# emanuele-artioli/elvis

Hardware: AMD Instinct MI355X
Metric: restored 1080p frames/sec, SinSR 4x path (ELVIS v2 Downsample) (higher is better)
Workload: dtype f16; 1 GPU; 30-frame 1920x1080 synthetic clip per GPU, ELVIS v2 Downsample (SinSR 4x), block 8, levels 0-3, weights seed 0 (random init), quantize=True; frames_per_gpu=30, parallelism=single GPU, gn_fused_into_conv=True, frames_per_invocation=15

## Files before the change

elvis_amd/_lib.py:

```python
from __future__ import annotations

import ctypes as C
import os
import threading
from typing import Optional

HERE = os.path.dirname(os.path.abspath(__file__))
LIBPATH = os.environ.get("ELVIS_AMD_LIB") or os.path.join(HERE, "lib", "libelvis_amd.so")

F32, F16 = 0, 1
ROUND_CV2, ROUND_HALF_UP = 0, 1

_lock = threading.Lock()
_lib: Optional[C.CDLL] = None

vp, i32, f32, i64, f64 = C.c_void_p, C.c_int, C.c_float, C.c_longlong, C.c_double


class ConvDesc(C.Structure):
    _fields_ = [(n, C.c_int) for n in (
        "dtype", "n", "h", "w", "cin", "cin_pitch", "cin2", "cin2_pitch", "cout", "cout_pitch",
        "ksize", "stride", "pad_before", "upsample", "ho", "wo", "act", "prologue", "subpixel")]


SIGNATURES = {
    "elvis_abi_version": [],
    "elvis_last_error": [],
    "elvis_last_launch": [],
    "elvis_recompose_u8": [vp, vp, vp, vp, vp, i32, i32, i32, i32, i32, i32, i32, i32, i32, vp],
    "elvis_area_downscale_u8": [vp, vp, i32, i32, i32, i32, i32, i32, vp],
    "elvis_blend_u8": [vp, vp, vp, vp, i32, i32, i32, i32, i32, i32, i32, f32, vp],
    "elvis_select_levels_u8": [vp, vp, i32, vp, vp, i32, i32, i32, i32, i32, i32, i32, vp],
    "elvis_tile_accumulate_f32": [vp, vp, vp, vp, vp, vp, i32, i32, i32, i32, i32, i32, i32, f32, vp],
    "elvis_tile_normalize_u8": [vp, vp, vp, i32, i32, i32, vp],
    "elvis_sse_u8": [vp, vp, vp, vp, vp, i32, i32, i32, i32, vp],
    "elvis_block_ssim_u8": [vp, vp, vp, vp, i32, i32, i32, i32, i32, vp],
    "elvis_u8_to_float": [vp, vp, i32, i32, i32, i32, i32, f32, f32, i32, i32, vp],
    "elvis_float_to_u8": [vp, i32, vp, vp, i32, i32, i32, i32, f32, f32, i32, i32, vp],
    "elvis_conv_packed_weight_bytes": [C.POINTER(ConvDesc)],
    "elvis_conv_pack_weights": [C.POINTER(ConvDesc), vp, vp, vp],
    "elvis_conv2d": [C.POINTER(ConvDesc), vp, vp, vp, vp, vp, i32, vp, vp, vp, vp, vp],
    "elvis_conv_stats_tiles": [C.POINTER(ConvDesc)],
    "elvis_conv_kernel_name": [C.POINTER(ConvDesc), C.c_char_p, C.c_size_t],
    "elvis_conv_kernel_name_for_call": [C.POINTER(ConvDesc), i32, i32, C.c_char_p, C.c_size_t],
    "elvis_conv_x3_eligible": [C.POINTER(ConvDesc)],
    "elvis_conv_debug_set": [C.c_char_p, i32],
    "elvis_gn_partials_to_sums": [vp, i32, i32, i32, vp, i32, i32, vp],
    "elvis_groupnorm_workspace_floats": [i32, i32, i32, i32],
    "elvis_groupnorm_sums": [vp, i32, i32, i32, i32, i32, vp, i32, i32, vp, vp],
    "elvis_groupnorm_affine": [vp, vp, vp, vp, vp, vp, vp, i32, i32, i32, i32, f32, vp],
    "elvis_affine_act": [vp, vp, i32, i32, i32, i32, i32, i32, vp, vp, i32, vp],
    "elvis_layernorm": [vp, vp, i32, i64, i32, i32, i32, vp, vp, f32, vp],
    "elvis_swin_packed_bytes": [i32, i32, i32],
    "elvis_swin_pack_weights": [vp, vp, vp, i32, i32, i32, vp],
    "elvis_swin_mlp": [vp, vp, vp, vp, vp, vp, vp, i64, i32, i32, i32, i32, f32, vp],
    "elvis_swin_ln_linear": [vp, vp, vp, vp, vp, vp, i64, i32, i32, i32, i32, f32, vp],
    "elvis_swin_pack_proj_mlp": [vp, vp, vp, vp, i32, i32, vp],
    "elvis_swin_proj_mlp": [vp, vp, vp, vp, vp, vp, vp, vp, vp, i64, i32, i32, i32, i32, i32, f32, vp],
    "elvis_window_attention": [vp, vp, i32, i32, i32, i32, i32, i32, i32, i32, i32, i32, vp, f32, vp],
    "elvis_bicubic_upsample": [vp, vp, i32, i32, i32, i32, i32, i32, i32, i32, vp],
    "elvis_vq_nearest": [vp, vp, vp, i32, i64, i32, i32, i32, vp, i32, vp],
    "elvis_pad_reflect_axpy": [vp, vp, i32, i32, i32, i32, i32, i32, i32, i32, i32, i32, f32, vp, f32, vp],
    "elvis_crop_copy": [vp, vp, i32, i32, i32, i32, i32, i32, i32, i32, i32, vp],
    "elvis_convert_act": [vp, i32, vp, i32, i64, i32, vp],
    "elvis_degrade_downsample_u8": [vp, vp, vp, i32, i32, i32, i32, i32, i32, i32, vp],
    "elvis_degrade_gaussian_u8": [vp, vp, vp, i32, i32, i32, i32, i32, i32, i32, f32, f32, f32, vp],
    "elvis_degrade_dct_u8": [vp, vp, vp, vp, vp, i32, i32, i32, i32, i32, i32, i32, vp],
    "elvis_degrade_scale_u8": [vp, vp, vp, i32, i32, i32, i32, i32, i32, i32, vp, vp, vp, i32, vp],
    "elvis_degrade_gaussian_fx_u8": [vp, vp, vp, i32, i32, i32, i32, i32, i32, i32, i32, i32, i32, vp],
    "elvis_classical_lanczos_u8": [vp, vp, vp, i32, i32, i32, i32, i32, i32, i32, vp, vp],
    "elvis_classical_unsharp_u8": [vp, vp, vp, i32, i32, i32, i32, i32, i32, i32, i32, vp, vp, i32, vp],
    "elvis_temporal_blend_u8": [vp, vp, i32, i64, f64, f64, vp],
    "elvis_block_gather_u8": [vp, vp, vp, vp, i32, i32, i32, i32, i32, i32, i32, i32, i32, vp],
    "elvis_shrink_select_topk": [vp, vp, vp, i32, i32, i32, i32, vp],
    "elvis_shrink_passes_plan": [i32, i32, i32, i32, vp, vp, vp, i32],
    "elvis_shrink_select_passes": [vp, vp, vp, vp, vp, vp, i32, i32, i32, i32, i32, i32, i32, vp],
    "elvis_stretch_index": [vp, vp, i32, i32, i32, i32, i32, i32, vp],
    "elvis_dcnv2": [vp, vp, vp, vp, vp, i32, i32, i32, i32, i32, i32, i32, i32, i32, i32, i32, i32, vp],
    "elvis_temporal_stack": [vp, vp, i32, i32, i32, i32, i32, i32, i32, i32, vp],
    "elvis_plane_merge": [vp, vp, vp, i32, i32, i32, i32, i32, i32, vp],
}


def lib() -> C.CDLL:
    global _lib
    if _lib is not None:
        return _lib
    with _lock:
        if _lib is not None:
            return _lib
        if not os.path.exists(LIBPATH):
            raise RuntimeError(
                f"libelvis_amd.so not found at {LIBPATH}. Build it with `python -m elvis_amd._build` "
                "(needs hipcc). There is no CPU fallback for the restoration path.")
        import torch
        try:
            handle = C.CDLL(LIBPATH)
        except OSError as exc:
            raise RuntimeError(f"failed to load {LIBPATH}: {exc}") from exc
        for name, argtypes in SIGNATURES.items():
            fn = getattr(handle, name)
            fn.argtypes = argtypes
            fn.restype = C.c_int
        handle.elvis_last_error.restype = C.c_char_p
        handle.elvis_last_launch.restype = C.c_char_p
        handle.elvis_conv_packed_weight_bytes.restype = C.c_size_t
        handle.elvis_groupnorm_workspace_floats.restype = C.c_size_t
        handle.elvis_swin_packed_bytes.restype = C.c_size_t
        if handle.elvis_abi_version() != 1:
            raise RuntimeError("libelvis_amd.so ABI version mismatch")
        _lib = handle
    return _lib


def check(rc: int, device=None) -> None:
    if rc == 0:
        return
    msg = lib().elvis_last_error().decode("utf-8", "replace")
    if rc == -1:
        raise ValueError(msg)
    label = str(device) if device is not None else "unknown device"
    raise RuntimeError(f"elvis_amd kernel failed on {label}: {msg}")


def ptr(t) -> int:
    return 0 if t is None else t.data_ptr()


def stream_handle(device=None) -> int:
    import torch
    return torch.cuda.current_stream(device).cuda_stream


def require_gpu(device) -> None:
    import torch
    dev = torch.device(device)
    if dev.type != "cuda":
        raise RuntimeError(
            f"elvis_amd runs on MI355X only (got device '{dev}'); there is no CPU path in the product. "
# ... 13 lines not shown
```

elvis_amd/csrc/conv.hip:

```cpp
#include "conv_kernels.inc"
#include "conv_ws.inc"
#include <string.h>

__attribute__((visibility("hidden"))) int elvis_conv_launch_f32_(const void* conv_args, int halo, int tco, int id, hipStream_t stream, void* query);
__attribute__((visibility("hidden"))) int elvis_conv_pack_x3p_(const float* w_oihw, void* packed, int cout, int ctot, int nkc, int n_co_tiles,
                                                              int tco, int taps, hipStream_t stream);

#include <atomic>
static std::atomic<int> g_no_halo{0};
static bool no_halo() { return g_no_halo.load(std::memory_order_relaxed) > 0; }
extern "C" int elvis_conv_debug_set(const char* key, int value) {
    ELVIS_REQUIRE(key, "elvis_conv_debug_set: null key");
    if (!strcmp(key, "no_halo")) { g_no_halo.store(value, std::memory_order_relaxed); return ELVIS_OK; }
    ELVIS_REQUIRE(false, "elvis_conv_debug_set: unknown key '%s'", key);
}

static void conv_geom(const elvis_conv_desc* d, int* nkc1, int* nkc, int* co_pad) {
    int kc = kc_of(d);
    *nkc1 = (d->cin + kc - 1) / kc;
    *nkc = *nkc1 + (d->cin2 > 0 ? (d->cin2 + kc - 1) / kc : 0);
    TileCfg t = choose_tile(d->cout);
    *co_pad = ((d->cout + t.tco - 1) / t.tco) * t.tco;
}

extern "C" size_t elvis_conv_packed_weight_bytes(const elvis_conv_desc* d) {
    if (!d || d->cin <= 0 || d->cout <= 0) return 0;
    int nkc1, nkc, co_pad;
    conv_geom(d, &nkc1, &nkc, &co_pad);
    return (size_t)d->ksize * d->ksize * nkc * co_pad * (x3_planar_fmt(d) ? 128 : 64);
}

extern "C" int elvis_conv_pack_weights(const elvis_conv_desc* d, const float* w_oihw, void* packed,
                                       elvis_stream_t stream) {
    int rc = validate(d);
    if (rc) return rc;
    ELVIS_REQUIRE(w_oihw && packed, "elvis_conv_pack_weights: null pointer");
    int nkc1, nkc, co_pad;
    conv_geom(d, &nkc1, &nkc, &co_pad);
    if (x3_planar_fmt(d)) {
        const int tco = choose_tile(d->cout).tco;
        return elvis_conv_pack_x3p_(w_oihw, packed, d->cout, d->cin + d->cin2, nkc, co_pad / tco, tco, d->ksize * d->ksize, (hipStream_t)stream);
    }
    int KC = kc_elems(d->dtype);
    long long total = (long long)d->ksize * d->ksize * nkc * co_pad * KC;
    int grid = (int)((total + 255) / 256);
    int ctot = d->cin + d->cin2;
// ... 18 lines not shown
}

enum class ConvPath { WS, HALO, IGEMM };
static ConvPath conv_path(const elvis_conv_desc* d, bool has_residual, bool has_stats) {
    if (no_halo()) return ConvPath::IGEMM;
    if (ws_shape_ok(d) && !has_residual && !has_stats) return ConvPath::WS;
    return halo_eligible(d) ? ConvPath::HALO : ConvPath::IGEMM;
}

static int conv_walk(const elvis_conv_desc* d, ConvPath path, const ConvArgs& a, hipStream_t stream, ConvPick* query) {
    const TileCfg t = choose_tile(d->cout);
    const bool f16 = d->dtype == ELVIS_F16;
    if (path == ConvPath::WS) return dispatch_ws(a, t.tco, stream, query);
    if (path == ConvPath::IGEMM) return f16 ? dispatch<half_t>(a, t.id, stream, query) : elvis_conv_launch_f32_(&a, 0, t.tco, t.id, stream, query);
    if (!f16) return elvis_conv_launch_f32_(&a, 1, t.tco, t.id, stream, query);
    switch (t.tco) {
        case 128: return launch_halo<half_t, 128>(a, stream, query);
        case 64: return launch_halo<half_t, 64>(a, stream, query);
        case 32: return launch_halo<half_t, 32>(a, stream, query);
        default: return launch_halo<half_t, 16>(a, stream, query);
    }
}

static int conv_plan(const elvis_conv_desc* d, ConvPath path, ConvArgs& a, ConvPick& pick) {
    a.n = d->n; a.h = d->h; a.w_in = d->w;
    a.cin = d->cin; a.cin_pitch = d->cin_pitch; a.cin2 = d->cin2; a.cin2_pitch = d->cin2_pitch;
    a.cout = d->cout; a.cout_pitch = d->cout_pitch;
    a.ksize = d->ksize; a.stride = d->stride; a.pad = d->pad_before; a.upsample = d->upsample;
    a.ho = d->ho; a.wo = d->wo; a.act = d->act; a.prologue = d->prologue;
    conv_geom(d, &a.nkc1, &a.nkc, &a.co_pad);
    TileCfg t = choose_tile(d->cout);
    a.M = (long long)d->n * d->ho * d->wo;
    a.n_co_tiles = a.co_pad / t.tco;
    a.n_px_tiles = (a.M + t.tpx - 1) / t.tpx;
    const bool s2d = d->ksize == 2 && d->subpixel == ELVIS_CONV_S2D;
    const bool subpix = d->ksize == 2 && !s2d;
    a.sub = d->ksize == 2;
    a.par_a = subpix ? (d->subpixel - 1) >> 1 : 0;
    a.par_b = subpix ? (d->subpixel - 1) & 1 : 0;
    a.ostr = subpix ? 2 : 1;
    a.pad2y = subpix ? 1 - a.par_a : (s2d ? d->pad_before : 0);
    a.pad2x = subpix ? 1 - a.par_b : (s2d ? d->pad_before : 0);
    a.s2d = s2d ? 1 : 0;
    a.istr = s2d ? 2 : 1;
    a.nkc_c = s2d ? d->cin / 4 / kc_of(d) : 0x3fffffff;
    a.wfull = d->w;
    if (s2d) {
        a.h = d->ho;
        a.w_in = d->wo;
    }
    a.x3 = d->dtype == ELVIS_F32X3 ? (x3_planar_run(d) ? 2 : 1) : 0;
    a.two = (halo_two(d) || halo_g1(d)) ? 1 : 0;
    a.tall = (halo_two(d) && halo_tall(d)) ? 1 : 0;
    int rc = conv_walk(d, path, a, nullptr, &pick);
    if (rc) return rc;
    a.tiles_x = ((subpix ? d->w : d->wo) + HALO_TX - 1) / HALO_TX;
    a.tiles_y = pick.ty > 0 ? ((subpix ? d->h : d->ho) + pick.ty - 1) / pick.ty : 0;
    a.strip = HALO_STRIP < a.tiles_x ? HALO_STRIP : 0;
    a.strip_full = a.strip > 0 ? a.tiles_x / a.strip : 0;
    return ELVIS_OK;
}

extern "C" int elvis_conv_stats_tiles(const elvis_conv_desc* d) {
    if (!d || !halo_eligible(d)) return 0;
    ConvArgs a{};
    ConvPick pick{};
    if (conv_plan(d, ConvPath::HALO, a, pick)) return 0;
    return d->n * a.tiles_y * a.tiles_x;
}

extern "C" int elvis_conv_kernel_name_for_call(const elvis_conv_desc* d, int has_residual, int has_stats, char* buf, size_t n) {
    int rc = validate(d);
    if (rc) return rc;
    ELVIS_REQUIRE(buf && n > 0, "elvis_conv_kernel_name: null buffer");
    ConvArgs a{};
    ConvPick pick{};
    rc = conv_plan(d, conv_path(d, has_residual != 0, has_stats != 0), a, pick);
    if (rc) return rc;
    snprintf(buf, n, "%s", pick.name);
    return ELVIS_OK;
}

extern "C" int elvis_conv_kernel_name(const elvis_conv_desc* d, char* buf, size_t n) {
    return elvis_conv_kernel_name_for_call(d, 0, 0, buf, n);
}

extern "C" int elvis_conv2d(const elvis_conv_desc* d, const void* x, const void* x2, const void* w_packed,
                            const float* bias, const void* residual, int residual_pitch, const float* pa,
                            const float* pb, void* out, float* stats, elvis_stream_t stream) {
    int rc = validate(d);
    if (rc) return rc;
    ELVIS_REQUIRE(x && w_packed && out, "elvis_conv2d: null pointer");
    ELVIS_REQUIRE(d->cin2 == 0 || x2, "elvis_conv2d: cin2 > 0 but x2 is null");
    ELVIS_REQUIRE(!d->prologue || (pa && pb), "elvis_conv2d: prologue requested without pa/pb");
    ELVIS_REQUIRE(d->dtype != ELVIS_F32X3 || x3_eligible(d),
                  "elvis_conv2d: this shape has no compensated-f16 kernel (elvis_conv_x3_eligible): run it as ELVIS_F32");
    ELVIS_REQUIRE(!residual || residual_pitch >= d->cout, "elvis_conv2d: bad residual pitch");
    ELVIS_REQUIRE(((uintptr_t)x | (uintptr_t)(x2 ? x2 : x) | (uintptr_t)w_packed | (uintptr_t)out) % 16 == 0,
                  "elvis_conv2d: pointers must be 16-byte aligned");
    const ConvPath path = conv_path(d, residual != nullptr, stats != nullptr);
    ELVIS_REQUIRE(path != ConvPath::IGEMM || !stats, "elvis_conv2d: fused statistics need a 3x3/stride-1 conv with cout >= 64 (query elvis_conv_stats_tiles)");
    ELVIS_REQUIRE(path == ConvPath::IGEMM || (long long)d->n * d->h * d->w < 0x7fffffffLL, "conv: input too large for 32-bit pixel indices");
    ConvArgs a{};
    ConvPick pick{};
    rc = conv_plan(d, path, a, pick);
    if (rc) return rc;
    a.x = x; a.x2 = x2; a.w = w_packed; a.bias = bias; a.res = residual; a.pa = pa; a.pb = pb; a.out = out;
    a.res_pitch = residual_pitch; a.stats = stats;
    return conv_walk(d, path, a, (hipStream_t)stream, nullptr);
}
```

elvis_amd/csrc/conv_kernels.inc:

```
#pragma once
#include "common.h"

#ifndef ELVIS_CONV_HOOKS
#define ELVIS_STAGE(x) x
#define ELVIS_STAGE_W(x) x
#define ELVIS_STAGE_H(x) x
#define ELVIS_SETPRIO(x)
#define ELVIS_BARRIER() __syncthreads()
#define ELVIS_HOOK_SKIP_STORE(tv)
#define ELVIS_HOOK_STAMP_BEGIN
#define ELVIS_HOOK_STAMP_LOOP
#define ELVIS_HOOK_STAMP_EPILOGUE
#define ELVIS_HOOK_STAMP_END
#endif

namespace {

struct ConvArgs {
    const void* x;
    const void* x2;
    const void* w;
    const float* bias;
    const void* res;
    const float* pa;
    const float* pb;
    void* out;
    int n, h, w_in;
    int cin, cin_pitch, cin2, cin2_pitch;
    int cout, cout_pitch, res_pitch;
    int ksize, stride, pad, upsample;
    int ho, wo;
    int act, prologue;
    int nkc;
    int nkc1;
    int co_pad;
    long long M;
    int n_co_tiles;
    long long n_px_tiles;
    int two, tall;
    float* stats;
    int tiles_x, tiles_y;
    int sub, par_a, par_b;
    int ostr, pad2y, pad2x;
    int s2d, istr, nkc_c, wfull;
    int strip;
    int strip_full;
    int x3;
};

struct ConvPick {
    const char* name;
    int ty;
    int set(const char* name_, int ty_) { name = name_; ty = ty_; return ELVIS_OK; }
};
constexpr const char* tf(bool b) { return b ? "true" : "false"; }

template <typename T> struct Frag;
template <> struct Frag<half_t> { typedef half8 type; };
template <> struct Frag<float> { typedef float4v type; };

__device__ __forceinline__ void mma_tile(float4v& acc, const half8& a, const half8& b) {
    acc = __builtin_amdgcn_mfma_f32_16x16x32_f16(a, b, acc, 0, 0, 0);
}
__device__ __forceinline__ void mma_tile(float4v& acc, const float4v& a, const float4v& b) {
    acc = __builtin_amdgcn_mfma_f32_16x16x4f32(a[0], b[0], acc, 0, 0, 0);
    acc = __builtin_amdgcn_mfma_f32_16x16x4f32(a[1], b[1], acc, 0, 0, 0);
    acc = __builtin_amdgcn_mfma_f32_16x16x4f32(a[2], b[2], acc, 0, 0, 0);
    acc = __builtin_amdgcn_mfma_f32_16x16x4f32(a[3], b[3], acc, 0, 0, 0);
}

__device__ __forceinline__ unsigned x3_pair(float v) {
    const half_t h = (half_t)v;
    const half_t l = (half_t)(v - (float)h);
    return (unsigned)__builtin_bit_cast(unsigned short, h) | ((unsigned)__builtin_bit_cast(unsigned short, l) << 16);
}
__device__ __forceinline__ uint4 x3_pair4(uint4 v) {
    return make_uint4(x3_pair(__builtin_bit_cast(float, v.x)), x3_pair(__builtin_bit_cast(float, v.y)),
                      x3_pair(__builtin_bit_cast(float, v.z)), x3_pair(__builtin_bit_cast(float, v.w)));
}
template <bool X3> __device__ __forceinline__ void mma_tile_x(float4v& acc, const half8& a, const half8& b) { mma_tile(acc, a, b); }
template <bool X3> __device__ __forceinline__ void mma_tile_x(float4v& acc, const float4v& a, const float4v& b) {
    if constexpr (X3) {
        const uint4 ap = __builtin_bit_cast(uint4, a);
        const uint4 a1 = make_uint4(__builtin_amdgcn_perm(ap.x, ap.x, 0x01000100u), __builtin_amdgcn_perm(ap.y, ap.y, 0x01000100u),
                                    __builtin_amdgcn_perm(ap.z, ap.z, 0x01000100u), __builtin_amdgcn_perm(ap.w, ap.w, 0x01000100u));
        const uint4 a2 = make_uint4(ap.x >> 16, ap.y >> 16, ap.z >> 16, ap.w >> 16);
        const half8 B = __builtin_bit_cast(half8, b);
        acc = __builtin_amdgcn_mfma_f32_16x16x32_f16(__builtin_bit_cast(half8, a1), B, acc, 0, 0, 0);
        acc = __builtin_amdgcn_mfma_f32_16x16x32_f16(__builtin_bit_cast(half8, a2), B, acc, 0, 0, 0);
    } else {
        mma_tile(acc, a, b);
    }
}

template <typename F> __device__ __forceinline__ F lds_frag(const char* p) {
    return *reinterpret_cast<const F*>(__builtin_assume_aligned(p, 16));
}

__device__ __forceinline__ int lds_row_off(int row, int q) {
    return row * 64 + ((q ^ (((row >> 2) & 1) << 1)) << 4);
}

constexpr int G1_NST128 = 3, G1_NST64 = 2;
typedef __attribute__((address_space(3))) void* lds_ptr_t;
typedef const __attribute__((address_space(1))) void* glb_ptr_t;

template <typename T> struct PrologueVec { float a[DT<T>::VEC], b[DT<T>::VEC]; };
template <typename T> __device__ __forceinline__ uint4 prologue_apply(uint4 v, const float (&pa)[DT<T>::VEC], const float (&pb)[DT<T>::VEC]);
template <> __device__ __forceinline__ uint4 prologue_apply<float>(uint4 v, const float (&pa)[4], const float (&pb)[4]) {
    float* f = reinterpret_cast<float*>(&v);
#pragma unroll
    for (int i = 0; i < 4; ++i) {
        float t = fmaf(f[i], pa[i], pb[i]);
        f[i] = t / (1.0f + expf(-t));
    }
    return v;
}
template <> __device__ __forceinline__ uint4 prologue_apply<half_t>(uint4 v, const float (&pa)[8], const float (&pb)[8]) {
    half_t* hv = reinterpret_cast<half_t*>(&v);
#pragma unroll
    for (int i = 0; i < 8; ++i) {
        float t = fmaf((float)hv[i], pa[i], pb[i]);
        hv[i] = (half_t)(t * __builtin_amdgcn_rcpf(1.0f + __expf(-t)));
    }
    return v;
}

__device__ __forceinline__ unsigned prologue_dword_f16(unsigned w, float a0, float a1, float b0, float b1, float K) {
    float u0, u1, e1;
    asm volatile(
        "v_fma_mix_f32 %1, %0, %4, %6 op_sel:[0,0,0] op_sel_hi:[1,0,0]\n\t"
        "v_fma_mix_f32 %2, %0, %5, %7 op_sel:[1,0,0] op_sel_hi:[1,0,0]\n\t"
        "v_exp_f32 %0, %1\n\t"
        "v_exp_f32 %3, %2\n\t"
        "v_fma_f32 %0, %0, %8, %8\n\t"
// ... 300 lines not shown
        }
    }
}

template <typename T, int TCO, int NT, int TY, bool PRO, int KS, bool ACT, bool X3>
__device__ __forceinline__ void conv3x3_halo_body(const ConvArgs& p) {
    constexpr int TX = 32, HX = TX + KS - 1, HY = TY + KS - 1, HP = HX * HY;
    constexpr bool TWO = NT == 256;
    constexpr int NSLOT = (TWO || KS == 2) ? 2 : 3;
    constexpr int NHB = TWO ? 1 : 2;
    constexpr bool WDMA = TWO;
    constexpr bool G1 = TWO && KS == 1;
    constexpr bool PSC = TWO && PRO && sizeof(T) == 2;
    constexpr int G1_NST = TCO == 64 ? G1_NST64 : G1_NST128;
    constexpr int HCH = HP * 4;
    constexpr int H_PER = (HCH + NT - 1) / NT;
    constexpr int HALO_BYTES = HP * 64;
    constexpr int W_TAP_BYTES = TCO * 64;
    constexpr int W_BYTES = KS * W_TAP_BYTES;
    constexpr int W_CHUNKS = W_TAP_BYTES / 16;
    constexpr int W_PER = (W_CHUNKS + NT - 1) / NT;
    constexpr int NW_CO = TCO >= 64 ? TCO / 64 : 1, NW_PX = (NT / 64) / NW_CO;
    constexpr int ROWS = TY / NW_PX;
    constexpr int WPX = ROWS * 2, WCO = TCO >= 64 ? 4 : TCO / 16;
    constexpr int VEC = DT<T>::VEC, KC = 4 * VEC;
    typedef typename Frag<T>::type frag_t;
    static_assert(ROWS * NW_PX == TY && ROWS >= 1, "tile rows must split evenly over the pixel waves");

    extern __shared__ __attribute__((aligned(16))) char smem[];
    char* const halo = smem;
    char* const wring = smem + NHB * HALO_BYTES;
    float* const ptab = reinterpret_cast<float*>(smem + NHB * HALO_BYTES + NSLOT * W_BYTES);

    const unsigned nblk = (unsigned)p.n_co_tiles * (unsigned)p.tiles_x * (unsigned)p.tiles_y * (unsigned)p.n;
    unsigned bid = blockIdx.x;
    {
        const unsigned q = nblk >> 3, r = nblk & 7u;
        const unsigned xcd = bid & 7u, idx = bid >> 3;
        bid = (xcd < r ? xcd * (q + 1) : r * (q + 1) + (xcd - r) * q) + idx;
    }
    int co_tile = 0;
    unsigned t = bid;
    if (p.n_co_tiles > 1) {
        t = bid / (unsigned)p.n_co_tiles;
        co_tile = (int)(bid - t * (unsigned)p.n_co_tiles);
    }
    int tx, ty, nimg;
    if (p.strip > 0) {
        const unsigned per_img = (unsigned)p.tiles_x * (unsigned)p.tiles_y;
        const unsigned ni = t / per_img;
        unsigned r = t - ni * per_img;
        const unsigned full = (unsigned)p.strip_full, strip_tiles = (unsigned)p.strip * (unsigned)p.tiles_y;
        unsigned s = r / strip_tiles;
        unsigned sw = (unsigned)p.strip;
        if (s >= full) { s = full; sw = (unsigned)p.tiles_x - full * (unsigned)p.strip; }
        r -= s * strip_tiles;
        const unsigned y = r / sw;
        nimg = (int)ni;
        ty = (int)y;
        tx = (int)(s * (unsigned)p.strip + (r - y * sw));
    } else {
        const unsigned row = t / (unsigned)p.tiles_x;
        tx = (int)(t - row * (unsigned)p.tiles_x);
        const unsigned ni = row / (unsigned)p.tiles_y;
        ty = (int)(row - ni * (unsigned)p.tiles_y);
        nimg = (int)ni;
    }
    const int oy0 = ty * TY, ox0 = tx * TX, co0 = co_tile * TCO;

    const int tid = threadIdx.x, lane = tid & 63, wave = tid >> 6;
    ELVIS_HOOK_STAMP_BEGIN
    const int w_co = wave / NW_PX, w_px = wave % NW_PX;
    const int lh = p.upsample ? p.h * 2 : p.h, lw = p.upsample ? p.w_in * 2 : p.w_in;

    const int pad_y = KS == 2 ? p.pad2y : KS / 2, pad_x = KS == 2 ? p.pad2x : KS / 2;
    int h_src[H_PER];
    unsigned h_ok = 0;
#pragma unroll
    for (int i = 0; i < H_PER; ++i) {
        int chunk = tid + i * NT;
        int pix = chunk >> 2;
        int hy = pix / HX, hx = pix - hy * HX;
        int gy = oy0 + hy - pad_y, gx = ox0 + hx - pad_x;
        bool ok = chunk < HCH && gy >= 0 && gy < lh && gx >= 0 && gx < lw;
        int sy = p.upsample ? (gy >> 1) : gy, sx = p.upsample ? (gx >> 1) : gx;
        h_src[i] = ok ? ((nimg * p.h + sy) * p.istr * p.w_in + sx) * p.istr : 0;
        h_ok |= (ok ? 1u : 0u) << i;
    }
    const bool halo_inside = oy0 - pad_y >= 0 && oy0 - pad_y + HY <= lh && ox0 - pad_x >= 0 && ox0 - pad_x + HX <= lw &&
                             (p.cin % KC) == 0 && (p.cin2 % KC) == 0 && p.cin_pitch >= p.nkc1 * KC && !(KS == 2 && p.s2d);
    const int q4 = tid & 3;
    const int nkc = p.nkc;
    const int nrows = nkc * KS;

    constexpr int HA = (H_PER + 1) / 2;
    uint4 hreg[H_PER];

    int wl_off[W_PER];
#pragma unroll
    for (int i = 0; i < W_PER; ++i) {
        int chunk = tid + i * NT;
        wl_off[i] = lds_row_off(chunk >> 2, chunk & 3);
    }

    auto chunk_c0 = [&](int kc, int& pixoff) -> int {
        pixoff = 0;
        if (KS == 2 && p.s2d) {
            const int ph = kc / p.nkc_c;
            pixoff = (ph >> 1) * p.wfull + (ph & 1);
            return (kc - ph * p.nkc_c) * KC + q4 * VEC;
        }
        return (kc >= p.nkc1 ? kc - p.nkc1 : kc) * KC + q4 * VEC;
    };
    auto halo_load = [&](int kc, int i0, int i1, bool live = true) {
        const bool second = kc >= p.nkc1;
        const char* xsrc = (const char*)(second ? p.x2 : p.x);
        const int pitch = second ? p.cin2_pitch : p.cin_pitch;
        int pixoff;
        const int c0 = chunk_c0(kc, pixoff);
        const int c0c = c0 < pitch ? c0 : 0;
// ... 10 lines not shown
        const bool ch_ok = c0 < pitch;
        char* dst = halo + buf * HALO_BYTES;
        float la[VEC], lb[VEC];
        if (PRO) {
            const float* tp = ptab + (kc * 4 + q4) * 2 * VEC;
#pragma unroll
            for (int e = 0; e < VEC; e += 4) {
                float4v a4 = *reinterpret_cast<const float4v*>(tp + e);
                float4v b4 = *reinterpret_cast<const float4v*>(tp + VEC + e);
#pragma unroll
                for (int k = 0; k < 4; ++k) { la[e + k] = a4[k]; lb[e + k] = b4[k]; }
            }
        }
#pragma unroll
        for (int i = i0; i < i1; ++i) {
            uint4 v = hreg[i];
            if constexpr (PSC) {
                const float K = -1.4426950408889634f;
                v.x = prologue_dword_f16(v.x, la[0], la[1], lb[0], lb[1], K);
                v.y = prologue_dword_f16(v.y, la[2], la[3], lb[2], lb[3], K);
                v.z = prologue_dword_f16(v.z, la[4], la[5], lb[4], lb[5], K);
                v.w = prologue_dword_f16(v.w, la[6], la[7], lb[6], lb[7], K);
            } else if (PRO) {
                v = prologue_apply<T>(v, la, lb);
            }
            if constexpr (X3) v = x3_pair4(v);
            if (!halo_inside) {
                const bool keep = ch_ok && ((h_ok >> i) & 1u);
                v.x = keep ? v.x : 0u; v.y = keep ? v.y : 0u; v.z = keep ? v.z : 0u; v.w = keep ? v.w : 0u;
            }
            int chunk = tid + i * NT;
            if ((i + 1) * NT <= HCH || chunk < HCH)
                *reinterpret_cast<uint4*>(dst + lds_row_off(chunk >> 2, chunk & 3)) = v;
        }
    };
    auto halo_act = [&](int kc, int slot, int half) {
        constexpr int HV = VEC / 2;
        const float* tp = ptab + (kc * 4 + q4) * 2 * VEC + half * HV;
        float a[HV], b[HV];
#pragma unroll
        for (int e = 0; e < HV; e += 2) {
            float2 a2 = *reinterpret_cast<const float2*>(tp + e);
            float2 b2 = *reinterpret_cast<const float2*>(tp + VEC + e);
            a[e] = a2.x; a[e + 1] = a2.y; b[e] = b2.x; b[e + 1] = b2.y;
        }
        uint2 v = half ? make_uint2(hreg[slot].z, hreg[slot].w) : make_uint2(hreg[slot].x, hreg[slot].y);
        v = prologue_apply_half(v, a, b, T());
        if (half) { hreg[slot].z = v.x; hreg[slot].w = v.y; } else { hreg[slot].x = v.x; hreg[slot].y = v.y; }
    };
    auto halo_write = [&](int kc, int buf, int slot) {
        const bool second = kc >= p.nkc1;
        const int pitch = second ? p.cin2_pitch : p.cin_pitch;
        int pixoff_;
        const int c0 = chunk_c0(kc, pixoff_);
        const bool keep = c0 < pitch && ((h_ok >> slot) & 1u);
        uint4 v = hreg[slot];
        if constexpr (X3) v = x3_pair4(v);
        v.x = keep ? v.x : 0u; v.y = keep ? v.y : 0u; v.z = keep ? v.z : 0u; v.w = keep ? v.w : 0u;
        int chunk = tid + slot * NT;
        if ((slot + 1) * NT <= HCH || chunk < HCH)
            *reinterpret_cast<uint4*>(halo + buf * HALO_BYTES + lds_row_off(chunk >> 2, chunk & 3)) = v;
    };
    static_assert(W_PER <= 2, "weight staging holds at most two 16-byte chunks per thread per tap");
    constexpr bool W_FULL0 = W_CHUNKS >= NT, W_FULL1 = W_PER == 2 && W_CHUNKS >= 2 * NT;
    const bool w_ok0 = W_FULL0 || tid < W_CHUNKS, w_ok1 = W_PER == 2 && (W_FULL1 || tid + NT < W_CHUNKS);
    uint4 wr00 = {}, wr01 = {}, wr10 = {}, wr11 = {}, wr20 = {}, wr21 = {};
// ... 648 lines not shown
        }
    } else
    if (p.stats) {
        float* red = reinterpret_cast<float*>(smem);
#pragma unroll
        for (int i = 0; i < WCO; ++i)
#pragma unroll
            for (int r = 0; r < 4; ++r) {
                const float a = row16_sum(st[i][r]), b = row16_sum(sq[i][r]);
                if (lr == 0) {
                    int cl = w_co * (16 * WCO) + cgrp * WCO + i * 4 + r;
                    red[(w_px * TCO + cl) * 2 + 0] = a;
                    red[(w_px * TCO + cl) * 2 + 1] = b;
                }
            }
        __syncthreads();
        if (tid < TCO && co0 + tid < p.cout) {
            float a = 0.f, b = 0.f;
#pragma unroll
            for (int w = 0; w < NW_PX; ++w) {
                a += red[(w * TCO + tid) * 2 + 0];
                b += red[(w * TCO + tid) * 2 + 1];
            }
            long long tile = ((long long)nimg * p.tiles_y + ty) * p.tiles_x + tx;
            float* dst = p.stats + (tile * p.cout + co0 + tid) * 2;
            dst[0] = a;
            dst[1] = b;
        }
    }
    ELVIS_HOOK_STAMP_END
}

template <typename T, int TCO, int NT, int TY, bool PRO, int KS = 3, bool ACT = false>
__global__ __launch_bounds__(NT, 2) void conv3x3_halo_kernel(ConvArgs p) {
    conv3x3_halo_body<T, TCO, NT, TY, PRO, KS, ACT, false>(p);
}
template <int TCO, int TY, bool PRO, int KS = 3, bool ACT = false>
__global__ __launch_bounds__(512, 2) void conv3x3_halo_x3_kernel(ConvArgs p) {
    conv3x3_halo_body<float, TCO, 512, TY, PRO, KS, ACT, true>(p);
}

struct TileCfg {
    int tco, tpx, id;
};
inline TileCfg choose_tile(int cout) {
    if (cout % 128 == 0) return {128, 128, 0};
    if (cout >= 64) return {64, 128, 1};
    if (cout <= 16) return {16, 256, 3};
    return {32, 256, 2};
}
inline bool halo_eligible(const elvis_conv_desc* d) {
    if (d->ksize == 2) return true;
    bool same = d->ho == (d->upsample ? 2 * d->h : d->h) && d->wo == (d->upsample ? 2 * d->w : d->w);
    if (d->ksize == 3) return d->stride == 1 && d->pad_before == 1 && same;
    return d->ksize == 1 && d->stride == 1 && d->pad_before == 0 && same && !d->prologue &&
           (long long)d->ho * d->wo >= 256;
}
constexpr int HALO_TY = 16, HALO_TY_PRO = 8, HALO_TY_PRO128 = 12, HALO_TX = 32;
constexpr int HALO_STRIP = 8;
constexpr int G1_TY128 = 8, G1_TY64 = 8;
constexpr int HALO_TY2 = 8, HALO_TY2_TALL = 16;
constexpr int X3P_TY128 = 12, X3P_TY64 = 16;

constexpr int halo_tile_rows(int ks, bool pro, int tco, int nt, bool tall) {
    if (nt == 256) return ks == 1 ? (tco == 128 ? G1_TY128 : G1_TY64) : tall ? HALO_TY2_TALL : HALO_TY2;
    if (ks == 3 && pro && tco == 128) return HALO_TY_PRO128;
    return (pro || ks == 1 || tco <= 32) ? HALO_TY_PRO : HALO_TY;
// ... 74 lines not shown
int launch(const ConvArgs& a, hipStream_t stream, ConvPick* query) {
    static const ElvisKernelName name("conv_igemm_kernel<%s,%d,%d,%d,%d>", sizeof(T) == 2 ? "half" : "float", WCO, WPX, NW_CO, NW_PX);
    if (query) return query->set(name.s, 0);
    constexpr int TCO = 16 * WCO * NW_CO, TPX = 16 * WPX * NW_PX;
    size_t lds = 2 * (size_t)(TCO + TPX) * 64;
    long long nblk = (long long)a.n_co_tiles * a.n_px_tiles;
    ELVIS_REQUIRE(nblk < 0x7fffffffLL, "conv: grid too large");
    hipLaunchKernelGGL((conv_igemm_kernel<T, WCO, WPX, NW_CO, NW_PX>), dim3((unsigned)nblk), dim3(64 * NW_CO * NW_PX),
                       lds, stream, a);
    ELVIS_CHECK_LAUNCH("elvis_conv2d");
    elvis_note_launch(name.s);
    return ELVIS_OK;
}

template <typename T, int TCO, bool PRO, int KS, int NT = 512, bool ACT = false, bool TALL = false, bool X3 = false>
int launch_halo_p(const ConvArgs& a, hipStream_t stream, ConvPick* query) {
    if constexpr (!ACT) {
        if (a.act != 0) return launch_halo_p<T, TCO, PRO, KS, NT, true, TALL, X3>(a, stream, query);
    }
    if constexpr (!X3 && sizeof(T) == 4 && NT == 512 && TCO >= 64) {
        if (a.x3) return launch_halo_p<T, TCO, PRO, KS, NT, ACT, TALL, true>(a, stream, query);
    }
    constexpr int TY = halo_tile_rows(KS, PRO, TCO, NT, TALL);
    static const ElvisKernelName name = X3 ? ElvisKernelName("conv3x3_halo_x3_kernel<%d,%d,%s,%d,%s>", TCO, TY, tf(PRO), KS, tf(ACT))
                                    : ElvisKernelName("conv3x3_halo_kernel<%s,%d,%d,%d,%s,%d,%s>", sizeof(T) == 2 ? "half" : "float", TCO, NT, TY, tf(PRO), KS, tf(ACT));
    if (query) return query->set(name.s, TY);
    const void* fn = nullptr;
    if constexpr (X3) fn = (const void*)conv3x3_halo_x3_kernel<TCO, TY, PRO, KS, ACT>;
    else fn = (const void*)conv3x3_halo_kernel<T, TCO, NT, TY, PRO, KS, ACT>;
    const size_t lds = halo_lds_bytes(KS, TCO, TY, NT, PRO ? a.nkc : 0, 4 * DT<T>::VEC);
    ELVIS_REQUIRE(lds <= 160 * 1024, "conv3x3_halo: %zu bytes of LDS needed (too many input channels)", lds);
    static ElvisLdsOptIn opt_in;
    if (int rc = elvis_lds_opt_in(fn, opt_in, elvis_device_slot(), "conv3x3_halo: cannot reserve %zu bytes of LDS", lds)) return rc;
    long long nblk = (long long)a.n_co_tiles * a.tiles_x * a.tiles_y * a.n;
    ELVIS_REQUIRE(nblk < 0x7fffffffLL, "conv: grid too large");
    if constexpr (X3) hipLaunchKernelGGL((conv3x3_halo_x3_kernel<TCO, TY, PRO, KS, ACT>), dim3((unsigned)nblk), dim3(NT), lds, stream, a);
    else hipLaunchKernelGGL((conv3x3_halo_kernel<T, TCO, NT, TY, PRO, KS, ACT>), dim3((unsigned)nblk), dim3(NT), lds, stream, a);
    ELVIS_CHECK_LAUNCH("elvis_conv2d(halo)");
    elvis_note_launch(name.s);
    return ELVIS_OK;
}

template <typename T, int TCO> int launch_halo(const ConvArgs& a, hipStream_t stream, ConvPick* query) {
    if constexpr (TCO >= 64 && sizeof(T) == 2) {
        if (a.two && a.ksize == 1) return launch_halo_p<T, TCO, false, 1, 256>(a, stream, query);
    }
    if (a.ksize == 1) return launch_halo_p<T, TCO, false, 1>(a, stream, query);
    if constexpr (TCO >= 64 && sizeof(T) == 2) {
        if (a.two && a.ksize == 2) return launch_halo_p<T, TCO, false, 2, 256>(a, stream, query);
        if constexpr (TCO == 64) {
            if (a.two && a.tall && a.ksize == 3)
                return a.prologue ? launch_halo_p<T, TCO, true, 3, 256, false, true>(a, stream, query)
                                  : launch_halo_p<T, TCO, false, 3, 256, false, true>(a, stream, query);
        }
        if (a.two) return a.prologue ? launch_halo_p<T, TCO, true, 3, 256>(a, stream, query) : launch_halo_p<T, TCO, false, 3, 256>(a, stream, query);
        ELVIS_REQUIRE(a.ksize == 3 && a.prologue, "conv3x3_halo: a conv without the prologue must fit the 256-thread kernel");
        return launch_halo_p<T, TCO, true, 3>(a, stream, query);
    } else {
        if (a.ksize == 2) return launch_halo_p<T, TCO, false, 2>(a, stream, query);
        return a.prologue ? launch_halo_p<T, TCO, true, 3>(a, stream, query) : launch_halo_p<T, TCO, false, 3>(a, stream, query);
    }
}

template <typename T> int dispatch(const ConvArgs& a, int id, hipStream_t stream, ConvPick* query) {
    switch (id) {
        case 0: return launch<T, 4, 4, 2, 2>(a, stream, query);
        case 1: return launch<T, 4, 2, 1, 4>(a, stream, query);
// ... 33 lines not shown
```

elvis_amd/ops.py:

```python
from __future__ import annotations

import ctypes as C
from dataclasses import dataclass
from typing import Optional

import torch

from . import _lib as L
from ._lib import ConvDesc, check, lib, ptr


def _s(t: torch.Tensor) -> int:
    return torch.cuda.current_stream(t.device).cuda_stream


def pitch_for(c: int) -> int:
    return (c + 7) // 8 * 8


@dataclass
class Act:
    t: torch.Tensor
    c: int
    stats: Optional[torch.Tensor] = None
# ... 192 lines not shown
            raise ValueError(f"conv: expected inputs with {self.cin}+{self.cin2} channels, got {x.c}+{x2.c if x2 else 0}")
        for t in (x, x2, residual):
            if t is not None and t.t.dtype != self.dtype:
                raise ValueError(f"conv: weights are packed for {self.dtype}, got a {t.t.dtype} tensor")
        d = ConvDesc()
        d.dtype = x.dtype_code
        d.n, d.h, d.w = x.n, x.h, x.w
        d.cin, d.cin_pitch = x.c, x.pitch
        d.cin2, d.cin2_pitch = (x2.c, x2.pitch) if x2 is not None else (0, 0)
        d.ksize, d.stride, d.upsample, d.act = self.ksize, stride, int(upsample), act
        d.pad_before = (self.ksize // 2) if pad is None else pad
        lh, lw = (x.h * 2, x.w * 2) if upsample else (x.h, x.w)
        if ho is None:
            ho = (lh + 2 * d.pad_before - self.ksize) // stride + 1
            wo = (lw + 2 * d.pad_before - self.ksize) // stride + 1
        d.ho, d.wo = ho, wo
        if out is None:
            out = new_act(x.n, ho, wo, self.cout, x.t.dtype, x.t.device, zero=False)
        d.cout, d.cout_pitch = self.cout_k, out.pitch
        pa = pb = None
        if prologue is not None:
            pa, pb = prologue
            d.prologue = 1
        stats = None
        packed = self.weights_for(d)
        tiles = lib().elvis_conv_stats_tiles(C.byref(d))
        if want_stats and tiles > 0:
            stats = torch.empty((tiles, self.cout_k, 2), dtype=torch.float32, device=x.t.device)
        out.stats = stats
        prof = CONV_PROFILER
        if prof is not None:
            e0, e1 = torch.cuda.Event(enable_timing=True), torch.cuda.Event(enable_timing=True)
            e0.record()
        check(lib().elvis_conv2d(C.byref(d), ptr(x.t), ptr(x2.t) if x2 is not None else 0, ptr(packed),
                                 ptr(self.bias), ptr(residual.t) if residual is not None else 0,
                                 residual.pitch if residual is not None else 0, ptr(pa), ptr(pb), ptr(out.t),
                                 ptr(stats), _s(x.t)), x.t.device)
        if prof is not None:
            e1.record()
            flops = 2.0 * self.ksize * self.ksize * (self.cin + self.cin2) * self.cout * x.n * ho * wo
            name = conv_kernel_name(d, residual=residual is not None, stats=stats is not None)
            if name.startswith("conv3x3_ws_kernel") and residual is None and KERNEL_PROFILER is not None:
                nbytes = float(self.cin + self.cin2 + self.cout) * x.t.element_size() * x.n * ho * wo
                KERNEL_PROFILER.append((name, "hbm", nbytes, e0, e1))
            else:
                prof.append((name, flops, e0, e1))
            if CONV_SHAPES is not None:
                CONV_SHAPES.append((x.n, x.h, x.w, self.cin + self.cin2, self.cout, self.ksize, stride,
                                    prologue is not None, residual is not None))
        if stats is not None and self.cout_k != self.cout:
            out.stats = stats[:, :self.cout].contiguous()
        return out


CONV_PROFILER = None
CONV_SHAPES = None
KERNEL_PROFILER = None


class _Timed:
    def __init__(self, name, bound, work):
        self.rec = (name, bound, work) if KERNEL_PROFILER is not None else None

    def __enter__(self):
        if self.rec:
            self.e0, self.e1 = torch.cuda.Event(enable_timing=True), torch.cuda.Event(enable_timing=True)
            self.e0.record()

    def __exit__(self, *exc):
        if self.rec and KERNEL_PROFILER is not None:
# ... 315 lines not shown
```

include/elvis_amd.h:

```cpp
#ifndef ELVIS_AMD_H
#define ELVIS_AMD_H

#include <stddef.h>
#include <stdint.h>

#ifdef __cplusplus
extern "C" {
#endif

#define ELVIS_ABI_VERSION 1

#define ELVIS_OK 0
#define ELVIS_E_INVALID (-1)
#define ELVIS_E_RUNTIME (-2)
#define ELVIS_E_UNSUPPORTED (-3)

#define ELVIS_F32 0
#define ELVIS_F16 1
#define ELVIS_F32X3 2

#define ELVIS_ROUND_CV2 0
#define ELVIS_ROUND_HALF_UP 1

typedef void* elvis_stream_t;
// ... 34 lines not shown
int elvis_u8_to_float(const uint8_t* src, void* dst, int dtype, int n, int h, int w, int pitch,
                      float scale, float bias, int swap_rb, int div255, elvis_stream_t stream);

int elvis_float_to_u8(const void* src, int dtype, uint8_t* dst, float* f32_out, int n, int h, int w,
                      int pitch, float scale, float bias, int mode, int swap_rb, elvis_stream_t stream);


typedef struct elvis_conv_desc {
    int dtype;
    int n, h, w;
    int cin, cin_pitch;
    int cin2, cin2_pitch;
    int cout, cout_pitch;
    int ksize;
    int stride;
    int pad_before;
    int upsample;
    int ho, wo;
    int act;
    int prologue;
    int subpixel;
} elvis_conv_desc;
#define ELVIS_CONV_S2D 5

size_t elvis_conv_packed_weight_bytes(const elvis_conv_desc* d);

int elvis_conv_pack_weights(const elvis_conv_desc* d, const float* w_oihw, void* packed,
                            elvis_stream_t stream);

int elvis_conv2d(const elvis_conv_desc* d, const void* x, const void* x2, const void* w_packed,
                 const float* bias, const void* residual, int residual_pitch, const float* pa,
                 const float* pb, void* out, float* stats, elvis_stream_t stream);

int elvis_conv_stats_tiles(const elvis_conv_desc* d);

int elvis_conv_kernel_name(const elvis_conv_desc* d, char* buf, size_t n);

int elvis_conv_kernel_name_for_call(const elvis_conv_desc* d, int has_residual, int has_stats, char* buf, size_t n);

int elvis_conv_debug_set(const char* key, int value);

int elvis_conv_x3_eligible(const elvis_conv_desc* d);

int elvis_gn_partials_to_sums(const float* partials, int tiles_per_image, int n, int c, double* sums,
                              int sums_ctot, int sums_coff, elvis_stream_t stream);

size_t elvis_groupnorm_workspace_floats(int dtype, int n, int hw, int c);
int elvis_groupnorm_sums(const void* x, int dtype, int n, int hw, int c, int pitch, double* sums,
                         int sums_ctot, int sums_coff, float* workspace, elvis_stream_t stream);

int elvis_groupnorm_affine(const double* sums, const float* gamma, const float* beta, const float* scale,
                           const float* shift, float* pa, float* pb, int n, int hw, int c, int groups,
                           float eps, elvis_stream_t stream);


int elvis_affine_act(const void* x, void* y, int dtype, int n, int hw, int c, int pitch_in,
                     int pitch_out, const float* pa, const float* pb, int act, elvis_stream_t stream);

int elvis_layernorm(const void* x, void* y, int dtype, long long tokens, int c, int pitch_in,
                    int pitch_out, const float* gamma, const float* beta, float eps, elvis_stream_t stream);

size_t elvis_swin_packed_bytes(int c, int n1, int mode);
int elvis_swin_pack_weights(const float* w1, const float* w2, void* packed, int c, int n1, int mlp, elvis_stream_t stream);
int elvis_swin_mlp(const void* x, void* out, const void* packed, const float* b1, const float* b2, const float* gamma,
                   const float* beta, long long tokens, int c, int hidden, int x_pitch, int out_pitch, float eps,
                   elvis_stream_t stream);
// ... 99 lines not shown
```

Baseline: 31.95 frames/s.

## Split prologue halo conv: first co-tile writes normalized activations, rest reuse them

For f16 3x3 halo convolutions that carry a GroupNorm/activation prologue and span several output-channel tiles, the conv now runs in two launches. The first computes only output-channel tile 0, applies the prologue, and also writes the normalized activations to a workspace. The second runs the remaining tiles without a prologue, reading that workspace. This removes the prologue arithmetic repeated in every co-tile block, at the cost of an extra activation write and read, a second launch, and a per-call torch allocation. Launch bounds for one kernel configuration also go from 2 to 3 blocks per SM.

New measurement: 31.60 frames/s. -1.1%, worse.

```diff
diff --git a/elvis_amd/_lib.py b/elvis_amd/_lib.py
--- a/elvis_amd/_lib.py
+++ b/elvis_amd/_lib.py
@@ -40,6 +40,8 @@
     "elvis_conv_packed_weight_bytes": [C.POINTER(ConvDesc)],
     "elvis_conv_pack_weights": [C.POINTER(ConvDesc), vp, vp, vp],
     "elvis_conv2d": [C.POINTER(ConvDesc), vp, vp, vp, vp, vp, i32, vp, vp, vp, vp, vp],
+    "elvis_conv_split_workspace_bytes": [C.POINTER(ConvDesc), i32, i32],
+    "elvis_conv2d_split": [C.POINTER(ConvDesc), vp, vp, vp, vp, vp, i32, vp, vp, vp, vp, vp, C.c_size_t, vp],
     "elvis_conv_stats_tiles": [C.POINTER(ConvDesc)],
     "elvis_conv_kernel_name": [C.POINTER(ConvDesc), C.c_char_p, C.c_size_t],
     "elvis_conv_kernel_name_for_call": [C.POINTER(ConvDesc), i32, i32, C.c_char_p, C.c_size_t],
@@ -105,6 +107,7 @@
         handle.elvis_last_error.restype = C.c_char_p
         handle.elvis_last_launch.restype = C.c_char_p
         handle.elvis_conv_packed_weight_bytes.restype = C.c_size_t
+        handle.elvis_conv_split_workspace_bytes.restype = C.c_size_t
         handle.elvis_groupnorm_workspace_floats.restype = C.c_size_t
         handle.elvis_swin_packed_bytes.restype = C.c_size_t
         if handle.elvis_abi_version() != 1:
diff --git a/elvis_amd/csrc/conv.hip b/elvis_amd/csrc/conv.hip
--- a/elvis_amd/csrc/conv.hip
+++ b/elvis_amd/csrc/conv.hip
@@ -7,11 +7,13 @@
                                                               int tco, int taps, hipStream_t stream);
 
 #include <atomic>
-static std::atomic<int> g_no_halo{0};
+static std::atomic<int> g_no_halo{0}, g_no_split{0};
 static bool no_halo() { return g_no_halo.load(std::memory_order_relaxed) > 0; }
+static bool no_split() { return g_no_split.load(std::memory_order_relaxed) > 0; }
 extern "C" int elvis_conv_debug_set(const char* key, int value) {
     ELVIS_REQUIRE(key, "elvis_conv_debug_set: null key");
     if (!strcmp(key, "no_halo")) { g_no_halo.store(value, std::memory_order_relaxed); return ELVIS_OK; }
+    if (!strcmp(key, "no_split")) { g_no_split.store(value, std::memory_order_relaxed); return ELVIS_OK; }
     ELVIS_REQUIRE(false, "elvis_conv_debug_set: unknown key '%s'", key);
 }
 
@@ -96,6 +98,7 @@
     TileCfg t = choose_tile(d->cout);
     a.M = (long long)d->n * d->ho * d->wo;
     a.n_co_tiles = a.co_pad / t.tco;
+    a.co_tile0 = 0; a.co_tiles = a.n_co_tiles;
     a.n_px_tiles = (a.M + t.tpx - 1) / t.tpx;
     const bool s2d = d->ksize == 2 && d->subpixel == ELVIS_CONV_S2D;
     const bool subpix = d->ksize == 2 && !s2d;
@@ -149,9 +152,50 @@
     return elvis_conv_kernel_name_for_call(d, 0, 0, buf, n);
 }
 
-extern "C" int elvis_conv2d(const elvis_conv_desc* d, const void* x, const void* x2, const void* w_packed,
-                            const float* bias, const void* residual, int residual_pitch, const float* pa,
-                            const float* pb, void* out, float* stats, elvis_stream_t stream) {
+struct ConvSplit {
+    elvis_conv_desc db;
+    ConvArgs a, b;
+    ConvPick pick_a, pick_b;
+    size_t bytes;
+};
+static bool halo_split(const elvis_conv_desc* d, int n_co_tiles) {
+    (void)d;
+    return n_co_tiles >= 2;
+}
+static int conv_split_plan(const elvis_conv_desc* d, bool has_residual, bool has_stats, ConvSplit& s) {
+    s.bytes = 0;
+    if (no_split() || d->dtype != ELVIS_F16 || d->ksize != 3 || !d->prologue || d->upsample) return ELVIS_OK;
+    if (conv_path(d, has_residual, has_stats) != ConvPath::HALO) return ELVIS_OK;
+    if (d->cin % 32 || d->cin2 % 32) return ELVIS_OK;
+    if ((long long)d->h * d->w * (d->cin + d->cin2) * 2 >= (1LL << 32)) return ELVIS_OK;
+    int rc = conv_plan(d, ConvPath::HALO, s.a, s.pick_a);
+    if (rc) return rc;
+    if (!s.a.two || !halo_split(d, s.a.n_co_tiles)) return ELVIS_OK;
+    s.db = *d;
+    s.db.prologue = 0;
+    s.db.cin = s.db.cin_pitch = d->cin + d->cin2;
+    s.db.cin2 = s.db.cin2_pitch = 0;
+    rc = conv_plan(&s.db, ConvPath::HALO, s.b, s.pick_b);
+    if (rc) return rc;
+    if (!s.b.two || s.pick_b.ty != s.pick_a.ty || s.b.nkc != s.a.nkc || !halo_co_window(256, 3, 2, false, s.pick_a.ty)) return ELVIS_OK;
+    s.a.co_tiles = 1;
+    s.a.act_pitch = s.db.cin;
+    s.b.co_tile0 = 1;
+    s.b.co_tiles = s.b.n_co_tiles - 1;
+    s.bytes = (size_t)d->n * d->h * d->w * s.db.cin * sizeof(half_t);
+    return ELVIS_OK;
+}
+
+extern "C" size_t elvis_conv_split_workspace_bytes(const elvis_conv_desc* d, int has_residual, int has_stats) {
+    if (!d || validate(d)) return 0;
+    ConvSplit s{};
+    if (conv_split_plan(d, has_residual != 0, has_stats != 0, s)) return 0;
+    return s.bytes;
+}
+
+static int conv2d_run(const elvis_conv_desc* d, const void* x, const void* x2, const void* w_packed,
+                      const float* bias, const void* residual, int residual_pitch, const float* pa,
+                      const float* pb, void* out, float* stats, void* workspace, size_t workspace_bytes, elvis_stream_t stream) {
     int rc = validate(d);
     if (rc) return rc;
     ELVIS_REQUIRE(x && w_packed && out, "elvis_conv2d: null pointer");
@@ -171,5 +215,40 @@
     if (rc) return rc;
     a.x = x; a.x2 = x2; a.w = w_packed; a.bias = bias; a.res = residual; a.pa = pa; a.pb = pb; a.out = out;
     a.res_pitch = residual_pitch; a.stats = stats;
+    if (workspace) {
+        ConvSplit s{};
+        rc = conv_split_plan(d, residual != nullptr, stats != nullptr, s);
+        if (rc) return rc;
+        if (s.bytes) {
+            ELVIS_REQUIRE(workspace_bytes >= s.bytes, "elvis_conv2d_split: workspace of %zu bytes, %zu needed (elvis_conv_split_workspace_bytes)",
+                          workspace_bytes, s.bytes);
+            ELVIS_REQUIRE((uintptr_t)workspace % 16 == 0, "elvis_conv2d_split: the workspace must be 16-byte aligned");
+            ELVIS_REQUIRE(workspace != x && workspace != x2 && workspace != out && workspace != residual,
+                          "elvis_conv2d_split: the workspace must not alias an input or the output");
+            s.a.x = x; s.a.x2 = x2; s.a.pa = pa; s.a.pb = pb; s.a.act_out = workspace;
+            s.b.x = workspace;
+            for (ConvArgs* l : {&s.a, &s.b}) {
+                l->w = w_packed; l->bias = bias; l->res = residual; l->res_pitch = residual_pitch; l->out = out; l->stats = stats;
+            }
+            rc = conv_walk(d, ConvPath::HALO, s.a, (hipStream_t)stream, nullptr);
+            if (rc) return rc;
+            rc = conv_walk(&s.db, ConvPath::HALO, s.b, (hipStream_t)stream, nullptr);
+            elvis_note_launch(s.pick_a.name);
+            return rc;
+        }
+    }
     return conv_walk(d, path, a, (hipStream_t)stream, nullptr);
 }
+
+extern "C" int elvis_conv2d(const elvis_conv_desc* d, const void* x, const void* x2, const void* w_packed,
+                            const float* bias, const void* residual, int residual_pitch, const float* pa,
+                            const float* pb, void* out, float* stats, elvis_stream_t stream) {
+    return conv2d_run(d, x, x2, w_packed, bias, residual, residual_pitch, pa, pb, out, stats, nullptr, 0, stream);
+}
+
+extern "C" int elvis_conv2d_split(const elvis_conv_desc* d, const void* x, const void* x2, const void* w_packed,
+                                  const float* bias, const void* residual, int residual_pitch, const float* pa,
+                                  const float* pb, void* out, float* stats, void* workspace, size_t workspace_bytes,
+                                  elvis_stream_t stream) {
+    return conv2d_run(d, x, x2, w_packed, bias, residual, residual_pitch, pa, pb, out, stats, workspace, workspace_bytes, stream);
+}
diff --git a/elvis_amd/csrc/conv_kernels.inc b/elvis_amd/csrc/conv_kernels.inc
--- a/elvis_amd/csrc/conv_kernels.inc
+++ b/elvis_amd/csrc/conv_kernels.inc
@@ -46,6 +46,9 @@
     int strip;
     int strip_full;
     int x3;
+    int co_tile0, co_tiles;
+    int act_pitch;
+    void* act_out;
 };
 
 struct ConvPick {
@@ -101,6 +104,7 @@
     return row * 64 + ((q ^ (((row >> 2) & 1) << 1)) << 4);
 }
 
+constexpr bool halo_co_window(int nt, int ks, int elem_bytes, bool x3, int ty) { return nt == 256 && ks == 3 && elem_bytes == 2 && !x3 && ty == 8; }
 constexpr int G1_NST128 = 3, G1_NST64 = 2;
 typedef __attribute__((address_space(3))) void* lds_ptr_t;
 typedef const __attribute__((address_space(1))) void* glb_ptr_t;
@@ -467,7 +471,9 @@
     char* const wring = smem + NHB * HALO_BYTES;
     float* const ptab = reinterpret_cast<float*>(smem + NHB * HALO_BYTES + NSLOT * W_BYTES);
 
-    const unsigned nblk = (unsigned)p.n_co_tiles * (unsigned)p.tiles_x * (unsigned)p.tiles_y * (unsigned)p.n;
+    constexpr bool CO_WIN = halo_co_window(NT, KS, sizeof(T), X3, TY);
+    const int n_co = CO_WIN ? p.co_tiles : p.n_co_tiles;
+    const unsigned nblk = (unsigned)n_co * (unsigned)p.tiles_x * (unsigned)p.tiles_y * (unsigned)p.n;
     unsigned bid = blockIdx.x;
     {
         const unsigned q = nblk >> 3, r = nblk & 7u;
@@ -476,10 +482,11 @@
     }
     int co_tile = 0;
     unsigned t = bid;
-    if (p.n_co_tiles > 1) {
-        t = bid / (unsigned)p.n_co_tiles;
-        co_tile = (int)(bid - t * (unsigned)p.n_co_tiles);
-    }
+    if (n_co > 1) {
+        t = bid / (unsigned)n_co;
+        co_tile = (int)(bid - t * (unsigned)n_co);
+    }
+    if constexpr (CO_WIN) co_tile += p.co_tile0;
     int tx, ty, nimg;
     if (p.strip > 0) {
         const unsigned per_img = (unsigned)p.tiles_x * (unsigned)p.tiles_y;
@@ -509,6 +516,9 @@
     const int lh = p.upsample ? p.h * 2 : p.h, lw = p.upsample ? p.w_in * 2 : p.w_in;
 
     const int pad_y = KS == 2 ? p.pad2y : KS / 2, pad_x = KS == 2 ? p.pad2x : KS / 2;
+    constexpr bool ACT_OUT = CO_WIN && PRO;
+    static_assert(H_PER <= 16, "h_ok holds two bits per staged chunk");
+    const bool act_on = ACT_OUT && p.act_out != nullptr;
     int h_src[H_PER];
     unsigned h_ok = 0;
 #pragma unroll
@@ -521,6 +531,10 @@
         int sy = p.upsample ? (gy >> 1) : gy, sx = p.upsample ? (gx >> 1) : gx;
         h_src[i] = ok ? ((nimg * p.h + sy) * p.istr * p.w_in + sx) * p.istr : 0;
         h_ok |= (ok ? 1u : 0u) << i;
+        if constexpr (ACT_OUT) {
+            const bool own = act_on && ok && hy >= pad_y && hy < pad_y + TY && hx >= pad_x && hx < pad_x + TX;
+            h_ok |= (own ? 1u : 0u) << (16 + i);
+        }
     }
     const bool halo_inside = oy0 - pad_y >= 0 && oy0 - pad_y + HY <= lh && ox0 - pad_x >= 0 && ox0 - pad_x + HX <= lw &&
                              (p.cin % KC) == 0 && (p.cin2 % KC) == 0 && p.cin_pitch >= p.nkc1 * KC && !(KS == 2 && p.s2d);
@@ -597,6 +611,22 @@
             int chunk = tid + i * NT;
             if ((i + 1) * NT <= HCH || chunk < HCH)
                 *reinterpret_cast<uint4*>(dst + lds_row_off(chunk >> 2, chunk & 3)) = v;
+            if constexpr (ACT_OUT) hreg[i] = v;
+        }
+        if constexpr (ACT_OUT) {
+            if (act_on) {
+                const int img0 = nimg * p.h * p.w_in;
+                char* const ob = (char*)p.act_out + (long long)img0 * p.act_pitch * (long long)sizeof(T);
+#pragma unroll
+                for (int i = i0; i < i1; ++i) {
+                    if ((h_ok >> (16 + i)) & 1u) {
+                        unsigned px = (unsigned)(h_src[i] - img0);
+                        asm volatile("" : "+v"(px));
+                        const unsigned off = (px * (unsigned)p.act_pitch + (unsigned)(kc * KC + q4 * VEC)) * (unsigned)sizeof(T);
+                        *reinterpret_cast<uint4*>(ob + off) = hreg[i];
+                    }
+                }
+            }
         }
     };
     auto halo_act = [&](int kc, int slot, int half) {
@@ -1311,7 +1341,7 @@
 }
 
 template <typename T, int TCO, int NT, int TY, bool PRO, int KS = 3, bool ACT = false>
-__global__ __launch_bounds__(NT, 2) void conv3x3_halo_kernel(ConvArgs p) {
+__global__ __launch_bounds__(NT, (NT == 256 && TCO == 64 && TY == 8 && KS == 3 && PRO && sizeof(T) == 2) ? 3 : 2) void conv3x3_halo_kernel(ConvArgs p) {
     conv3x3_halo_body<T, TCO, NT, TY, PRO, KS, ACT, false>(p);
 }
 template <int TCO, int TY, bool PRO, int KS = 3, bool ACT = false>
@@ -1452,7 +1482,7 @@
     ELVIS_REQUIRE(lds <= 160 * 1024, "conv3x3_halo: %zu bytes of LDS needed (too many input channels)", lds);
     static ElvisLdsOptIn opt_in;
     if (int rc = elvis_lds_opt_in(fn, opt_in, elvis_device_slot(), "conv3x3_halo: cannot reserve %zu bytes of LDS", lds)) return rc;
-    long long nblk = (long long)a.n_co_tiles * a.tiles_x * a.tiles_y * a.n;
+    long long nblk = (long long)(halo_co_window(NT, KS, sizeof(T), X3, TY) ? a.co_tiles : a.n_co_tiles) * a.tiles_x * a.tiles_y * a.n;
     ELVIS_REQUIRE(nblk < 0x7fffffffLL, "conv: grid too large");
     if constexpr (X3) hipLaunchKernelGGL((conv3x3_halo_x3_kernel<TCO, TY, PRO, KS, ACT>), dim3((unsigned)nblk), dim3(NT), lds, stream, a);
     else hipLaunchKernelGGL((conv3x3_halo_kernel<T, TCO, NT, TY, PRO, KS, ACT>), dim3((unsigned)nblk), dim3(NT), lds, stream, a);
diff --git a/elvis_amd/ops.py b/elvis_amd/ops.py
--- a/elvis_amd/ops.py
+++ b/elvis_amd/ops.py
@@ -248,10 +248,13 @@
         if prof is not None:
             e0, e1 = torch.cuda.Event(enable_timing=True), torch.cuda.Event(enable_timing=True)
             e0.record()
-        check(lib().elvis_conv2d(C.byref(d), ptr(x.t), ptr(x2.t) if x2 is not None else 0, ptr(packed),
-                                 ptr(self.bias), ptr(residual.t) if residual is not None else 0,
-                                 residual.pitch if residual is not None else 0, ptr(pa), ptr(pb), ptr(out.t),
-                                 ptr(stats), _s(x.t)), x.t.device)
+        ws_bytes = lib().elvis_conv_split_workspace_bytes(C.byref(d), int(residual is not None), int(stats is not None))
+        ws = torch.empty(ws_bytes, dtype=torch.uint8, device=x.t.device) if ws_bytes else None
+        check(lib().elvis_conv2d_split(C.byref(d), ptr(x.t), ptr(x2.t) if x2 is not None else 0, ptr(packed),
+                                       ptr(self.bias), ptr(residual.t) if residual is not None else 0,
+                                       residual.pitch if residual is not None else 0, ptr(pa), ptr(pb), ptr(out.t),
+                                       ptr(stats), ptr(ws), ws_bytes, _s(x.t)), x.t.device)
+        del ws
         if prof is not None:
             e1.record()
             flops = 2.0 * self.ksize * self.ksize * (self.cin + self.cin2) * self.cout * x.n * ho * wo
diff --git a/include/elvis_amd.h b/include/elvis_amd.h
--- a/include/elvis_amd.h
+++ b/include/elvis_amd.h
@@ -90,6 +90,12 @@
                  const float* bias, const void* residual, int residual_pitch, const float* pa,
                  const float* pb, void* out, float* stats, elvis_stream_t stream);
 
+size_t elvis_conv_split_workspace_bytes(const elvis_conv_desc* d, int has_residual, int has_stats);
+int elvis_conv2d_split(const elvis_conv_desc* d, const void* x, const void* x2, const void* w_packed,
+                       const float* bias, const void* residual, int residual_pitch, const float* pa,
+                       const float* pb, void* out, float* stats, void* workspace, size_t workspace_bytes,
+                       elvis_stream_t stream);
+
 int elvis_conv_stats_tiles(const elvis_conv_desc* d);
 
 int elvis_conv_kernel_name(const elvis_conv_desc* d, char* buf, size_t n);
```
